# gattia/pyfocusr

Measured on AMD Instinct MI355X. Metric: lowest-k eigenpairs/sec + KNN-correspondence wall-clock, 250k-vertex mesh pair k=5, higher is better.
Workload: dtype f64

## Files before the change

### include/pyfocusr_hip.h

```cpp
#ifndef PYFOCUSR_HIP_H
#define PYFOCUSR_HIP_H

#include <stddef.h>
#include <stdint.h>

#ifdef __cplusplus
extern "C" {
#endif

#define PF_VERSION 1

#define PF_OK 0
#define PF_E_ARG (-1)
#define PF_E_HIP (-2)
#define PF_E_DEGENERATE (-3)
#define PF_E_STATE (-4)
#define PF_E_PERSIST_TIMEOUT (-5)
#define PF_E_INTERNAL (-6)

#define PF_OP_RW 0
#define PF_OP_SYM 1

typedef struct pf_ctx pf_ctx;
typedef struct pf_graph pf_graph;
// ... 97 lines not shown
int pf_orth_end(pf_graph* g, double* h, double* nrm);
int pf_orth_begin2(pf_graph* ga, int32_t w_a, int32_t first_a, int32_t count_a, int32_t normalize_a, pf_graph* gb, int32_t w_b,
                   int32_t first_b, int32_t count_b, int32_t normalize_b);
int pf_orth_cheb2(pf_graph* ga, pf_graph* gb, const int32_t* orth, const int32_t* cheb_i, const double* cheb_d);
int pf_orth_redone(pf_graph* g);
int pf_orth_strict(pf_graph* g, int32_t on);
int pf_orth_device_passes(pf_graph* g, int32_t on);
int pf_orth_split(pf_graph* g, int32_t first2, int32_t split);
int pf_orth_one_launch(int32_t on);
int pf_scale(pf_graph* g, int32_t slot, double alpha);
int pf_combine(pf_graph* g, int32_t src_first, int32_t m, const double* Y, int32_t k, int32_t dst_first);
int pf_resnorm(pf_graph* g, int32_t ax, int32_t x, double lam, double* out);
int pf_gram(pf_graph* g, int32_t first_a, int32_t count_a, int32_t first_b, int32_t count_b, double* out);
int pf_resnorms(pf_graph* g, int32_t ax_first, int32_t x_first, const double* lam, int32_t count, double* out);
int pf_finalize_vectors(pf_graph* g, int32_t first, int32_t count, int32_t from_sym, int32_t minmax,
                        double* out);
int pf_finalize_vectors_begin(pf_graph* g, int32_t first, int32_t count, int32_t from_sym, int32_t minmax, double* out);
int pf_finalize_vectors_end(pf_graph* g);
int pf_final_remap_begin(pf_graph* g, const int32_t* col, const double* sign, int32_t count, double* out);
int pf_host_alloc(size_t bytes, void** out);
int pf_host_free(void* p);
int pf_host_detach(void* p);
int pf_final_rows(pf_graph* g, const int64_t* rows, int64_t n_rows, double* out);
int pf_point_rows(pf_graph* g, const int64_t* rows, int64_t n_rows, double* out);
int pf_spmv_host(pf_graph* g, int32_t op, const double* x, double* y);
int pf_mean_filter(pf_graph* g, const double* values, int32_t ncols, int32_t iterations, double* out);

int pf_knn1(pf_ctx* ctx, const double* ref, int64_t n_ref, const double* qry, int64_t n_qry, int32_t d,
            int64_t* idx_out, double* d2_out);
int pf_knn_mode(pf_ctx* ctx, int32_t mode);
int pf_knn_tree_stats(pf_ctx* ctx, int32_t enable_counting, int64_t* leaves_scanned, int64_t* supers_opened);
int pf_knn_count(pf_ctx* ctx, int32_t enable_counting, int64_t* pairs);
int pf_knn_wave_stats(pf_ctx* ctx, double* sum_us, double* max_us, int64_t* waves, int64_t* max_candidates, double* detail);
int pf_knn(pf_ctx* ctx, const double* ref, int64_t n_ref, const double* qry, int64_t n_qry, int32_t d, int32_t k,
           int64_t* idx_out, double* d2_out);
int pf_knn_topk(pf_ctx* ctx, const double* ref, int64_t n_ref, const double* qry, int64_t n_qry, int32_t d, int32_t k,
                int64_t* idx_out, double* d2_out);
int pf_knn1_graphs(pf_graph* ref_g, pf_graph* qry_g, int32_t d, const int32_t* col_ref, const double* scale_ref,
                   const int32_t* col_qry, const double* scale_qry, int64_t* idx_out, double* d2_out);
int pf_knn1_blocks(pf_ctx* ctx, const double* ref_block, int64_t n_ref, int32_t ref_stride, const double* qry_block,
                   int64_t n_qry, int32_t qry_stride, int32_t d, const int32_t* col_ref, const double* scale_ref,
                   const int32_t* col_qry, const double* scale_qry, int64_t* idx_out, double* d2_out);
int pf_eigsort_costs(pf_graph* g_target, pf_graph* g_source, const int64_t* rows_t, int64_t m_t, const int64_t* rows_s, int64_t m_s,
                     int32_t k, const int32_t* col_t, const double* sign_t, const int32_t* col_s, const double* sign_s, double* out,
                     int64_t* idx_out);
int pf_final_device(pf_graph* g, double** block, int64_t* n_rows, int32_t* n_cols);
int pf_knn_upload(pf_ctx* ctx, const double* ref, int64_t n_ref, const double* qry, int64_t n_qry, int32_t d);
int pf_knn_run(pf_ctx* ctx);
int pf_knn_download(pf_ctx* ctx, int64_t* idx_out, double* d2_out);

int pf_knn1_wide(pf_ctx* ctx, const double* ref, int64_t n_ref, const double* qry, int64_t n_qry, int32_t d,
                 int64_t* idx_out, double* d2_out );
int pf_knn1_wide_count(pf_ctx* ctx, int32_t enable_counting, int64_t* coordinate_pairs);
typedef struct pf_fmap pf_fmap;
int pf_fmap_create(pf_ctx* ctx, const double* phi_t, int64_t n_t, const double* phi_s, int64_t n_s, const double* mass_s,
                   int32_t K, pf_fmap** out);
void pf_fmap_free(pf_fmap* h);
int pf_fmap_set_p2p(pf_fmap* h, const int64_t* T);
int pf_fmap_get_p2p(pf_fmap* h, int64_t* T_out, double* d2_out);
int pf_fmap_project(pf_fmap* h, int32_t k_s, int32_t k_t, double* C_out);
int pf_fmap_convert(pf_fmap* h, const double* C, int32_t k_s, int32_t k_t);
int pf_fmap_zoomout(pf_fmap* h, int32_t k_start, int32_t k_end, int32_t step, int32_t n_iter_at_end, double* C_out);
int pf_fmap_set_samples(pf_fmap* h, const int64_t* S_t, int64_t q_t, const int64_t* S_s, int64_t q_s);
int pf_fmap_zoomout_sampled(pf_fmap* h, int32_t k_start, int32_t k_end, int32_t step, int32_t n_iter_at_end, double* C_out);

int pf_fps(pf_ctx* ctx, const double* points, int64_t n, int32_t d, int64_t m, int64_t start, int64_t* sel_out,
// ... 129 lines not shown
```

### pyfocusr_amd/_hip.py

```python
import atexit
import ctypes as C
import os
import threading
import weakref

import numpy as np

_HERE = os.path.dirname(os.path.abspath(__file__))
LIB_PATH = os.environ.get("PYFOCUSR_HIP_LIB", os.path.join(_HERE, "csrc", "libpyfocusr_hip.so"))

PF_OP_RW = 0
PF_OP_SYM = 1

_f64p = C.POINTER(C.c_double)
_i32p = C.POINTER(C.c_int32)
_i64p = C.POINTER(C.c_int64)


class HipUnavailable(RuntimeError):
    pass


class PfError(RuntimeError):
    def __init__(self, code, msg):
# ... 93 lines not shown
    "pf_eigsort_costs": (C.c_int, [C.c_void_p, C.c_void_p, _i64p, C.c_int64, _i64p, C.c_int64, C.c_int32, _i32p, _f64p, _i32p, _f64p, _f64p,
                                   _i64p]),
    "pf_orth_redone": (C.c_int, [C.c_void_p]),
    "pf_orth_strict": (C.c_int, [C.c_void_p, C.c_int32]),
    "pf_scale": (C.c_int, [C.c_void_p, C.c_int32, C.c_double]),
    "pf_combine": (C.c_int, [C.c_void_p, C.c_int32, C.c_int32, _f64p, C.c_int32, C.c_int32]),
    "pf_resnorm": (C.c_int, [C.c_void_p, C.c_int32, C.c_int32, C.c_double, _f64p]),
    "pf_gram": (C.c_int, [C.c_void_p, C.c_int32, C.c_int32, C.c_int32, C.c_int32, _f64p]),
    "pf_resnorms": (C.c_int, [C.c_void_p, C.c_int32, C.c_int32, _f64p, C.c_int32, _f64p]),
    "pf_finalize_vectors": (C.c_int, [C.c_void_p, C.c_int32, C.c_int32, C.c_int32, C.c_int32, _f64p]),
    "pf_finalize_vectors_begin": (C.c_int, [C.c_void_p, C.c_int32, C.c_int32, C.c_int32, C.c_int32, _f64p]),
    "pf_finalize_vectors_end": (C.c_int, [C.c_void_p]),
    "pf_final_remap_begin": (C.c_int, [C.c_void_p, _i32p, _f64p, C.c_int32, _f64p]),
    "pf_host_alloc": (C.c_int, [C.c_size_t, C.POINTER(C.c_void_p)]),
    "pf_host_free": (C.c_int, [C.c_void_p]),
    "pf_final_rows": (C.c_int, [C.c_void_p, _i64p, C.c_int64, _f64p]),
    "pf_point_rows": (C.c_int, [C.c_void_p, _i64p, C.c_int64, _f64p]),
    "pf_spmv_host": (C.c_int, [C.c_void_p, C.c_int32, _f64p, _f64p]),
    "pf_mean_filter": (C.c_int, [C.c_void_p, _f64p, C.c_int32, C.c_int32, _f64p]),
    "pf_knn1": (C.c_int, [C.c_void_p, _f64p, C.c_int64, _f64p, C.c_int64, C.c_int32, _i64p, _f64p]),
    "pf_knn": (C.c_int, [C.c_void_p, _f64p, C.c_int64, _f64p, C.c_int64, C.c_int32, C.c_int32, _i64p, _f64p]),
    "pf_knn_topk": (C.c_int, [C.c_void_p, _f64p, C.c_int64, _f64p, C.c_int64, C.c_int32, C.c_int32, _i64p, _f64p]),
    "pf_knn1_graphs": (C.c_int, [C.c_void_p, C.c_void_p, C.c_int32, _i32p, _f64p, _i32p, _f64p, _i64p, _f64p]),
    "pf_knn1_blocks": (C.c_int, [C.c_void_p, C.c_void_p, C.c_int64, C.c_int32, C.c_void_p, C.c_int64, C.c_int32, C.c_int32,
                                 _i32p, _f64p, _i32p, _f64p, _i64p, _f64p]),
    "pf_final_device": (C.c_int, [C.c_void_p, C.POINTER(C.c_void_p), _i64p, _i32p]),
    "pf_knn_upload": (C.c_int, [C.c_void_p, _f64p, C.c_int64, _f64p, C.c_int64, C.c_int32]),
    "pf_knn_run": (C.c_int, [C.c_void_p]),
    "pf_knn_download": (C.c_int, [C.c_void_p, _i64p, _f64p]),
    "pf_eigs_smallest": (C.c_int, [C.c_void_p, C.c_int32, C.c_int32, _f64p, _f64p, C.POINTER(C.c_int32), C.POINTER(EigsStats)]),
    "pf_knn_count": (C.c_int, [C.c_void_p, C.c_int32, C.POINTER(C.c_int64)]),
    "pf_knn_wave_stats": (C.c_int, [C.c_void_p, C.POINTER(C.c_double), C.POINTER(C.c_double), C.POINTER(C.c_int64), C.POINTER(C.c_int64),
                                    _f64p]),
    "pf_host_detach": (C.c_int, [C.c_void_p]),
    "pf_orth_device_passes": (C.c_int, [C.c_void_p, C.c_int32]),
    "pf_eigs_smallest_ex": (C.c_int, [C.c_void_p, C.c_int32, C.c_int32, C.c_int32, _f64p, _f64p, _f64p, C.POINTER(C.c_int32),
                                      C.POINTER(EigsStats)]),
    "pf_eigs_smallest2": (C.c_int, [C.c_void_p, C.c_void_p, C.c_int32, C.c_int32, C.c_int32, C.c_int32,
                                    _f64p, _f64p, _f64p, C.POINTER(C.c_int32), C.POINTER(EigsStats),
                                    _f64p, _f64p, _f64p, C.POINTER(C.c_int32), C.POINTER(EigsStats)]),
    "pf_op_step": (C.c_int, [C.c_void_p, C.c_int32, C.c_int32, C.c_int32, C.c_int32, C.c_double, C.c_double, C.c_double]),
    "pf_cheb_steps": (C.c_int, [C.c_void_p, C.c_int32, C.c_int32, C.c_int32, C.c_int32, C.c_int32, C.c_double, C.c_double,
                                C.c_double, C.POINTER(C.c_int32), C.POINTER(C.c_int32)]),
    "pf_axpy": (C.c_int, [C.c_void_p, C.c_int32, C.c_int32, C.c_int32, _f64p]),
    "pf_rows_create": (C.c_int, [C.c_void_p, _i64p, C.c_int64, C.POINTER(C.c_void_p)]),
    "pf_rows_free": (None, [C.c_void_p]),
    "pf_rows_gather": (C.c_int, [C.c_void_p, C.c_int32, _f64p]),
    "pf_rows_scatter": (C.c_int, [C.c_void_p, C.c_int32, _f64p]),
    "pf_rows_gather_dev": (C.c_int, [C.c_void_p, C.c_int32, C.c_void_p]),
    "pf_rows_scatter_dev": (C.c_int, [C.c_void_p, C.c_int32, C.c_void_p]),
    "pf_rows_set_sources": (C.c_int, [C.c_void_p, _i64p]),
    "pf_rows_gather2_dev": (C.c_int, [C.c_void_p, C.c_int32, C.c_int32, C.c_void_p, C.c_int64]),
    "pf_rows_scatter2_dev": (C.c_int, [C.c_void_p, C.c_int32, C.c_int32, C.c_void_p, C.c_int64]),
    "pf_rows_fill": (C.c_int, [C.c_void_p, C.c_int32, C.c_double]),
    "pf_surface_create": (C.c_int, [C.c_void_p, _f64p, C.c_int64, _i32p, C.c_int64, C.c_int32, C.POINTER(C.c_void_p)]),
    "pf_surface_free": (None, [C.c_void_p]),
    "pf_surface_closest": (C.c_int, [C.c_void_p, _f64p, C.c_int64, _f64p, _i32p, _f64p]),
    "pf_surface_distance": (C.c_int, [C.c_void_p, _f64p, C.c_int64, _f64p, _i32p, _f64p]),
    "pf_surface_prepare_signed": (C.c_int, [C.c_void_p, _f64p, _i32p, _i64p]),
    "pf_surface_signed_distance": (C.c_int, [C.c_void_p, _f64p, C.c_int64, _f64p, _i32p, _i32p, _i64p]),
    "pf_surface_prepare_winding": (C.c_int, [C.c_void_p]),
    "pf_surface_winding": (C.c_int, [C.c_void_p, _f64p, C.c_int64, C.c_double, _f64p, _f64p]),
    "pf_surface_raycast": (C.c_int, [C.c_void_p, _f64p, _f64p, C.c_int64, C.c_double, C.c_double, C.c_int32, _f64p, _i32p, _f64p,
                                     _i32p]),
    "pf_surface_vertex_normals": (C.c_int, [C.c_void_p, _f64p]),
    "pf_knn1_wide": (C.c_int, [C.c_void_p, _f64p, C.c_int64, _f64p, C.c_int64, C.c_int32, _i64p, _f64p]),
# ... 320 lines not shown
                child.close()
            self._lib.pf_destroy(self._h)
            self._h = None

    def __del__(self):
        try:
            self.close()
        except Exception:
            pass

    def sync(self):
        _check(self._lib.pf_sync(self._h))

    @property
    def stream_ptr(self):
        return int(self._lib.pf_stream(self._h) or 0)

    def timing_enable(self, on=True):
        _check(self._lib.pf_timing_enable(self._h, int(on)))

    def timing(self, reset=False):
        t = Timing()
        _check(self._lib.pf_timing_get(self._h, C.byref(t), int(bool(reset))))
        return t.as_dict()

    def knn_mode(self, mode):
        _check(self._lib.pf_knn_mode(self._h, int(mode)))

    def knn_count(self, enable_counting=False):
        pairs = C.c_int64()
        _check(self._lib.pf_knn_count(self._h, int(bool(enable_counting)), C.byref(pairs)))
        return int(pairs.value)

    def knn_tree_stats(self, enable_counting=False):
        a, b = C.c_int64(), C.c_int64()
        _check(self._lib.pf_knn_tree_stats(self._h, int(bool(enable_counting)), C.byref(a), C.byref(b)))
        return int(a.value), int(b.value)

    def knn1(self, ref, qry, return_d2=False):
        ref, qry = _same_d(ref, qry)
        idx = np.empty(qry.shape[0], dtype=np.int64)
        d2 = np.empty(qry.shape[0], dtype=np.float64) if return_d2 else None
        _check(self._lib.pf_knn1(self._h, _f64(ref), ref.shape[0], _f64(qry), qry.shape[0], ref.shape[1],
                                 _ptr(idx), _f64(d2)))
        return (idx, d2) if return_d2 else idx

    def knn1_wide(self, ref, qry, return_d2=False):
        ref, qry = _same_d(ref, qry)
        idx = np.empty(qry.shape[0], dtype=np.int64)
        d2 = np.empty(qry.shape[0], dtype=np.float64) if return_d2 else None
        _check(self._lib.pf_knn1_wide(self._h, _f64(ref), ref.shape[0], _f64(qry), qry.shape[0], ref.shape[1],
                                      _ptr(idx), _f64(d2)))
        return (idx, d2) if return_d2 else idx

    def knn1_wide_count(self, enable_counting=False):
        pairs = C.c_int64()
        _check(self._lib.pf_knn1_wide_count(self._h, int(bool(enable_counting)), C.byref(pairs)))
        return int(pairs.value)

    def farthest_point_sampling(self, points, m, start=-1, return_owner=False, return_d2=False):
        pts = _c_f64(points)
        if pts.ndim != 2:
            raise ValueError("points must be an (n, d) array")
        n, m = pts.shape[0], int(m)
        sel = np.empty(max(m, 0), dtype=np.int64)
        owner = np.empty(n, dtype=np.int32) if return_owner else None
# ... 915 lines not shown
```

### pyfocusr_amd/csrc/pf_knn.hip

```cpp
#include <hipcub/hipcub.hpp>

#include <string.h>

#include <algorithm>

#include "pf_internal.h"
#include "pf_wave.h"

namespace {

constexpr int KNN_LDS_DOUBLES = 4096;

struct KnnGrid {
    int a0, a1;
    int r0, r1;
    double lo0, lo1;
    double s0, s1;
};

__device__ __forceinline__ int cell_of(double x, double lo, double scale, int r) {
    const double t = (x - lo) * scale;
    return t > 0.0 ? (t >= (double)r ? r - 1 : (int)t) : 0;
}

__global__ __launch_bounds__(PF_BLOCK) void k_extent(const double* __restrict__ pts, int64_t n, int d, unsigned long long* ext ) {
    __shared__ unsigned long long part[PF_BLOCK / PF_WAVE][32];
    const int wave = threadIdx.x / PF_WAVE;
    for (int a = 0; a < d; ++a) {
        unsigned long long lo = ~0ull, hi = 0ull;
        for (int64_t i = (int64_t)blockIdx.x * PF_BLOCK + threadIdx.x; i < n; i += (int64_t)gridDim.x * PF_BLOCK) {
            const unsigned long long e = enc_f64(pts[i * d + a]);
            lo = e < lo ? e : lo;
            hi = e > hi ? e : hi;
        }
        for (int off = PF_WAVE / 2; off > 0; off >>= 1) {
            const unsigned long long l2 = __shfl_xor(lo, off, PF_WAVE), h2 = __shfl_xor(hi, off, PF_WAVE);
            lo = l2 < lo ? l2 : lo;
            hi = h2 > hi ? h2 : hi;
// ... 19 lines not shown
    }
}

__global__ void k_make_grid(const unsigned long long* __restrict__ ext, int d, int res, KnnGrid* g) {
    if (threadIdx.x | blockIdx.x) return;
    int b0 = 0, b1 = 0;
    double w0 = -1.0, w1 = -1.0;
    for (int a = 0; a < d; ++a) {
        const double e = dec_f64(ext[16 + a]) - dec_f64(ext[a]);
        if (e > w0) {
            w1 = w0;
            b1 = b0;
            w0 = e;
            b0 = a;
        } else if (e > w1) {
            w1 = e;
            b1 = a;
        }
    }
    if (d == 1) {
        b1 = b0;
        w1 = 0.0;
    }
    g->a0 = b0;
    g->a1 = b1;
    g->r0 = res;
    g->r1 = d == 1 ? 1 : res;
    g->lo0 = dec_f64(ext[b0]);
    g->lo1 = dec_f64(ext[b1]);
    g->s0 = (w0 > 0.0 && isfinite(w0)) ? (double)res / w0 : 0.0;
    g->s1 = (d > 1 && w1 > 0.0 && isfinite(w1)) ? (double)res / w1 : 0.0;
}

__device__ __forceinline__ unsigned spread16(unsigned v) {
    v &= 0xffffu;
    v = (v | (v << 8)) & 0x00ff00ffu;
    v = (v | (v << 4)) & 0x0f0f0f0fu;
    v = (v | (v << 2)) & 0x33333333u;
    v = (v | (v << 1)) & 0x55555555u;
    return v;
}

__global__ __launch_bounds__(PF_BLOCK) void k_cell_keys(const double* __restrict__ pts, int64_t n, int d,
                                                        const KnnGrid* __restrict__ gp, int morton, unsigned* __restrict__ keys,
                                                        int32_t* __restrict__ vals, int32_t* __restrict__ hist) {
    const int64_t i = (int64_t)blockIdx.x * PF_BLOCK + threadIdx.x;
    if (i >= n) return;
    const KnnGrid g = *gp;
    const int cx = cell_of(pts[i * d + g.a0], g.lo0, g.s0, g.r0);
    const int cy = cell_of(pts[i * d + g.a1], g.lo1, g.s1, g.r1);
    const unsigned key = morton ? (spread16((unsigned)cx) | (spread16((unsigned)cy) << 1)) : (unsigned)(cy * g.r0 + cx);
    keys[i] = key;
    if (hist) atomicAdd(&hist[key], 1);
    else vals[i] = (int32_t)i;
}

__global__ __launch_bounds__(PF_BLOCK) void k_gather_rows(const double* __restrict__ pts, const int32_t* __restrict__ order,
                                                          int64_t n, int d, double* __restrict__ out) {
    const int64_t i = (int64_t)blockIdx.x * PF_BLOCK + threadIdx.x;
    if (i >= n) return;
    const int64_t src = order[i];
    for (int c = 0; c < d; ++c) out[i * d + c] = pts[src * d + c];
}

__global__ __launch_bounds__(PF_BLOCK) void k_cell_start(const unsigned* __restrict__ keys, int64_t n, int64_t n_cells,
                                                         int32_t* __restrict__ cell_start) {
    const int64_t c = (int64_t)blockIdx.x * PF_BLOCK + threadIdx.x;
    if (c > n_cells) return;
    int64_t lo = 0, hi = n;
    while (lo < hi) {
        const int64_t mid = (lo + hi) >> 1;
        if ((int64_t)keys[mid] < c) lo = mid + 1; else hi = mid;
    }
    cell_start[c] = (int32_t)lo;
}

template <int D>
__device__ __forceinline__ double dist2(const double (&q)[D], const double* __restrict__ r) {
    double s = 0.0;
#pragma unroll
    for (int c = 0; c < D; ++c) {
        const double df = q[c] - r[c];
        const double sq = df * df;
        s = (c == 0) ? sq : s + sq;
// ... 190 lines not shown
                    s = dist2<D>(q, tile + r * D);
                }
                if (s <= bestk[K - 1]) {
                    const int32_t o = tile_idx[r];
                    bool seen = false;
#pragma unroll
                    for (int j = 0; j < K; ++j) seen |= (bidx[j] == o);
                    if (!seen) topk_insert<K>(bestk, bidx, s, o);
                }
            }
        }
        since_refresh += run_e - run_b;
        if (since_refresh >= 4 * KNN_TILE && by1 - by0 >= 8) {
            since_refresh = 0;
            int nx0, nx1, ny0, ny1;
            block_rectangle(nx0, nx1, ny0, ny1);
            bx0 = max(bx0, nx0);
            bx1 = min(bx1, nx1);
            by0 = max(by0, ny0);
            by1 = min(by1, ny1);
        }
    }
    if (mine) {
        const int64_t dst = qry_orig[qi];
#pragma unroll
        for (int j = 0; j < K; ++j) {
            idx_out[dst * K + j] = bidx[j];
            d2_out[dst * K + j] = bestk[j];
        }
    }
}

constexpr int knn_group(int d) { return d <= 4 ? 8 : (d <= 8 ? 4 : 2); }

template <int D, bool COUNT = false>
__global__ __launch_bounds__(PF_BLOCK) void k_knn_coop(const double* __restrict__ soa, int64_t ld, const int32_t* __restrict__ ref_orig,
                                                       const int32_t* __restrict__ cell_start, const double* __restrict__ qry_s,
                                                       const int32_t* __restrict__ qry_orig, int64_t n_qry,
                                                       const KnnGrid* __restrict__ gp, int64_t* __restrict__ idx_out,
                                                       double* __restrict__ d2_out, unsigned long long* __restrict__ visited = nullptr) {
    constexpr int G = knn_group(D);
    unsigned long long seen = 0;
    const unsigned long long t_begin = COUNT ? __builtin_amdgcn_s_memrealtime() : 0ull;
    unsigned long long n_chunks = 0, n_scans = 0, t_scan = 0, t_bounds = 0, n_pass = 0;
    const KnnGrid g = *gp;
    const int lane = threadIdx.x & (PF_WAVE - 1);
    const int64_t group = (int64_t)blockIdx.x * (PF_BLOCK / PF_WAVE) + __builtin_amdgcn_readfirstlane((int)(threadIdx.x / PF_WAVE));
    const int64_t q0 = group * G;
    if (q0 >= n_qry) return;
    const int nq = n_qry - q0 < G ? (int)(n_qry - q0) : G;
    double q[G][D];
    double qx[G], qy[G];
    double best[G];
    int32_t bidx[G];
    int ux0 = 0x7fffffff, ux1 = -1, uy0 = 0x7fffffff, uy1 = -1;
#pragma unroll
    for (int i = 0; i < G; ++i) {
        const int64_t qi = q0 + (i < nq ? i : nq - 1);
#pragma unroll
        for (int c = 0; c < D; ++c) q[i][c] = qry_s[qi * D + c];
        qx[i] = qry_s[qi * D + g.a0];
        qy[i] = qry_s[qi * D + g.a1];
        const int cx = cell_of(qx[i], g.lo0, g.s0, g.r0), cy = cell_of(qy[i], g.lo1, g.s1, g.r1);
        ux0 = min(ux0, cx), ux1 = max(ux1, cx);
        uy0 = min(uy0, cy), uy1 = max(uy1, cy);
        best[i] = INFINITY;
        bidx[i] = 0x7fffffff;
    }
    auto scan_rows = [&](int row_of, int x0, int x1) {
        int32_t b_l = 0, e_l = 0;
        if (row_of >= 0) {
            b_l = cell_start[row_of * g.r0 + x0];
            e_l = cell_start[row_of * g.r0 + x1 + 1];
        }
        int32_t inc = (e_l - b_l + PF_WAVE - 1) >> 6;
#pragma unroll
        for (int off = 1; off < PF_WAVE; off <<= 1) {
            const int32_t up = __shfl_up(inc, off, PF_WAVE);
            if (lane >= off) inc += up;
        }
        const int32_t total = __builtin_amdgcn_readlane(inc, PF_WAVE - 1);
        if constexpr (COUNT) n_chunks += (unsigned long long)total, n_scans += 1ull;
        for (int32_t j = 0; j < total; ++j) {
            const int row = (int)__popcll(__ballot(inc <= j));
            const int32_t first = row > 0 ? __builtin_amdgcn_readlane(inc, row - 1) : 0;
            const int32_t r = __builtin_amdgcn_readlane(b_l, row) + (j - first) * PF_WAVE + lane;
            if constexpr (COUNT) seen += (unsigned long long)__popcll(__ballot(r < __builtin_amdgcn_readlane(e_l, row)));
            if (r < __builtin_amdgcn_readlane(e_l, row)) {
                double x[D];
#pragma unroll
                for (int c = 0; c < D; ++c) x[c] = soa[(int64_t)c * ld + r];
                const int32_t o = ref_orig[r];
                if constexpr (COUNT) {
                    bool pass = false;
#pragma unroll
                    for (int i = 0; i < G; ++i) {
                        double s3 = 0.0;
#pragma unroll
                        for (int c = 0; c < D; ++c)
                            if (c != g.a0 && c != g.a1) s3 += (q[i][c] - x[c]) * (q[i][c] - x[c]);
                        pass = pass || s3 <= best[i];
                    }
                    n_pass += (unsigned long long)__popcll(__ballot(pass));
                }
#pragma unroll
                for (int i = 0; i < G; ++i) {
                    double s = 0.0;
                    constexpr int P = D >= 6 ? D / 2 : D;
#pragma unroll
                    for (int c = 0; c < P; ++c) {
                        const double df = q[i][c] - x[c];
                        const double sq = df * df;
                        s = (c == 0) ? sq : s + sq;
                    }
                    if constexpr (P < D) {
                        if (!__any(s <= best[i])) continue;
#pragma unroll
                        for (int c = P; c < D; ++c) {
                            const double df = q[i][c] - x[c];
                            s = s + df * df;
                        }
                    }
                    if (s < best[i] || (s == best[i] && o < bidx[i])) {
                        best[i] = s;
                        bidx[i] = o;
                    }
                }
            }
        }
    };
    auto bounds = [&](int& bx0, int& bx1, int& by0, int& by1) -> bool {
        bool all = true;
        bx0 = 0x7fffffff, bx1 = -1, by0 = 0x7fffffff, by1 = -1;
#pragma unroll
        for (int i = 0; i < G; ++i) {
            wave_argmin(best[i], bidx[i]);
            all = all && best[i] < INFINITY;
            const double rad = sqrt(best[i]) * (1.0 + 1e-9) + 1e-300;
            double xl = qx[i] - rad, xh = qx[i] + rad, yl = qy[i] - rad, yh = qy[i] + rad;
            xl -= fabs(xl) * 1e-15;
            xh += fabs(xh) * 1e-15;
            yl -= fabs(yl) * 1e-15;
            yh += fabs(yh) * 1e-15;
            bx0 = min(bx0, cell_of(xl, g.lo0, g.s0, g.r0)), bx1 = max(bx1, cell_of(xh, g.lo0, g.s0, g.r0));
            by0 = min(by0, cell_of(yl, g.lo1, g.s1, g.r1)), by1 = max(by1, cell_of(yh, g.lo1, g.s1, g.r1));
        }
        if (!all) bx0 = 0, by0 = 0, bx1 = g.r0 - 1, by1 = g.r1 - 1;
        return all;
    };
    int x0 = 0, x1 = -1, y0 = 0, y1 = -1;
    int rx0 = 0, rx1 = -1, ry0 = 0, ry1 = -1;
    for (int ring = 1; ring <= 4; ++ring) {
        rx0 = max(ux0 - ring, 0), rx1 = min(ux1 + ring, g.r0 - 1);
        ry0 = max(uy0 - ring, 0), ry1 = min(uy1 + ring, g.r1 - 1);
        unsigned long long ta = COUNT ? __builtin_amdgcn_s_memrealtime() : 0ull;
        for (int yb = ry0; yb <= ry1; yb += PF_WAVE) scan_rows(yb + lane <= ry1 ? yb + lane : -1, rx0, rx1);
        unsigned long long tb = COUNT ? __builtin_amdgcn_s_memrealtime() : 0ull;
        const bool all_bounded = bounds(x0, x1, y0, y1);
        if constexpr (COUNT) t_scan += tb - ta, t_bounds += __builtin_amdgcn_s_memrealtime() - tb;
        if (all_bounded) break;
    }
    if (!(x0 >= rx0 && x1 <= rx1 && y0 >= ry0 && y1 <= ry1)) {
        const int mid = min(max((uy0 + uy1) / 2, y0), y1);
        int lo = mid, hi = mid - 1;
        int w = 4;
        while (lo > y0 || hi < y1) {
            const int na = max(min(w, y1 - hi), 0), nb = max(min(w, lo - y0), 0);
            unsigned long long ta = COUNT ? __builtin_amdgcn_s_memrealtime() : 0ull;
            scan_rows(lane < na ? hi + 1 + lane : (lane < na + nb ? lo - 1 - (lane - na) : -1), x0, x1);
            unsigned long long tb = COUNT ? __builtin_amdgcn_s_memrealtime() : 0ull;
            hi += na;
            lo -= nb;
            w = min(2 * w, PF_WAVE / 2);
            int nx0, nx1, ny0, ny1;
            bounds(nx0, nx1, ny0, ny1);
            if constexpr (COUNT) t_scan += tb - ta, t_bounds += __builtin_amdgcn_s_memrealtime() - tb;
            x0 = max(x0, nx0), x1 = min(x1, nx1);
            y0 = max(y0, ny0), y1 = min(y1, ny1);
        }
    }
#pragma unroll
    for (int i = 0; i < G; ++i) {
        if (lane == i && i < nq) {
            const int64_t dst = qry_orig[q0 + i];
            idx_out[dst] = bidx[i];
            d2_out[dst] = best[i];
        }
    }
    if constexpr (COUNT) {
        if (lane == 0 && visited) {
            atomicAdd(visited, seen * (unsigned long long)nq);
            unsigned long long* rec = visited + 8 + 8 * group;
            rec[0] = __builtin_amdgcn_s_memrealtime() - t_begin;
            rec[1] = seen;
            rec[2] = n_chunks;
            rec[3] = n_scans;
            rec[4] = t_scan;
            rec[5] = t_bounds;
            rec[6] = n_pass;
        }
    }
}

constexpr int64_t PF_KNN_SMALL = 16384;
constexpr int knn_small_group(int d) { return d <= 4 ? 8 : 4; }

template <int D>
__global__ __launch_bounds__(PF_BLOCK) void k_knn_small(const double* __restrict__ ref, int64_t n_ref, const double* __restrict__ qry,
                                                        int64_t n_qry, int64_t* __restrict__ idx_out, double* __restrict__ d2_out) {
    constexpr int G = knn_small_group(D);
    const int lane = threadIdx.x & (PF_WAVE - 1);
    const int64_t group = (int64_t)blockIdx.x * (PF_BLOCK / PF_WAVE) + __builtin_amdgcn_readfirstlane((int)(threadIdx.x / PF_WAVE));
    const int64_t q0 = group * G;
    if (q0 >= n_qry) return;
    const int nq = n_qry - q0 < G ? (int)(n_qry - q0) : G;
    double q[G][D], best[G];
    int32_t bidx[G];
#pragma unroll
    for (int i = 0; i < G; ++i) {
        const int64_t qi = q0 + (i < nq ? i : nq - 1);
#pragma unroll
        for (int c = 0; c < D; ++c) q[i][c] = qry[qi * D + c];
        best[i] = INFINITY;
        bidx[i] = 0x7fffffff;
    }
    for (int64_t r = lane; r < n_ref; r += PF_WAVE) {
        double x[D];
#pragma unroll
        for (int c = 0; c < D; ++c) x[c] = ref[r * D + c];
#pragma unroll
        for (int i = 0; i < G; ++i) {
            double s = 0.0;
// ... 11 lines not shown
    }
#pragma unroll
    for (int i = 0; i < G; ++i) {
        wave_argmin(best[i], bidx[i]);
        if (lane == i && i < nq) {
            idx_out[q0 + i] = bidx[i];
            d2_out[q0 + i] = best[i];
        }
    }
}

template <int D>
static int launch_knn_small(pf_ctx* c) {
    const int64_t groups = (c->knn_nqry + knn_small_group(D) - 1) / knn_small_group(D);
    k_knn_small<D><<<(unsigned)((groups + PF_BLOCK / PF_WAVE - 1) / (PF_BLOCK / PF_WAVE)), PF_BLOCK, 0, c->stream>>>(
        c->knn_ref.p, c->knn_nref, c->knn_qry.p, c->knn_nqry, c->knn_idx.p, c->knn_d2.p);
    PF_HIP(hipGetLastError());
    return PF_OK;
}

__global__ __launch_bounds__(PF_BLOCK) void k_gather_rows_soa(const double* __restrict__ pts, const int32_t* __restrict__ order,
                                                              int64_t n, int d, int64_t ld, double* __restrict__ out) {
    const int64_t i = (int64_t)blockIdx.x * PF_BLOCK + threadIdx.x;
    if (i >= n) return;
    const int64_t src = order[i];
    for (int c = 0; c < d; ++c) out[(int64_t)c * ld + i] = pts[src * d + c];
}

template <int D, int K>
int launch_knn_k(pf_ctx* c) {
    constexpr int BS = D <= 6 ? PF_WAVE : PF_BLOCK;
    if constexpr (K == 1 && D <= 9) {
        const int64_t waves = (c->knn_nqry + knn_group(D) - 1) / knn_group(D);
        if (c->knn_count_on) {
            const int64_t words = 8 + 8 * waves;
            PF_HIP(c->knn_visited.grow(c->stream, words));
            c->knn_visited_waves = waves;
            PF_HIP(hipMemsetAsync(c->knn_visited.p, 0, words * sizeof(unsigned long long), c->stream));
            k_knn_coop<D, true><<<(unsigned)((waves + PF_BLOCK / PF_WAVE - 1) / (PF_BLOCK / PF_WAVE)), PF_BLOCK, 0, c->stream>>>(
                c->knn_ref_soa.p, c->knn_ref_ld, c->knn_ref_orig.p, c->knn_cell_start.p, c->knn_qry_s.p, c->knn_qry_orig.p, c->knn_nqry,
                (const KnnGrid*)c->knn_grid, c->knn_idx.p, c->knn_d2.p, c->knn_visited.p);
        } else {
            k_knn_coop<D><<<(unsigned)((waves + PF_BLOCK / PF_WAVE - 1) / (PF_BLOCK / PF_WAVE)), PF_BLOCK, 0, c->stream>>>(
                c->knn_ref_soa.p, c->knn_ref_ld, c->knn_ref_orig.p, c->knn_cell_start.p, c->knn_qry_s.p, c->knn_qry_orig.p, c->knn_nqry,
                (const KnnGrid*)c->knn_grid, c->knn_idx.p, c->knn_d2.p);
        }
    } else {
        k_knn_grid<D, K, BS, 512><<<(unsigned)((c->knn_nqry + BS - 1) / BS), BS, 0, c->stream>>>(
            c->knn_ref_s.p, c->knn_ref_orig.p, c->knn_cell_start.p, c->knn_nref, c->knn_qry_s.p, c->knn_qry_orig.p, c->knn_nqry,
            (const KnnGrid*)c->knn_grid, c->knn_idx.p, c->knn_d2.p);
    }
    PF_HIP(hipGetLastError());
    return PF_OK;
}

template <int D>
int launch_knn(pf_ctx* c) {
    if (c->knn_k == 1) return launch_knn_k<D, 1>(c);
    if constexpr (D <= 4) {
        if (c->knn_k == 2) return launch_knn_k<D, 2>(c);
        if (c->knn_k == 3) return launch_knn_k<D, 3>(c);
        if (c->knn_k == 4) return launch_knn_k<D, 4>(c);
    }
    pf_set_error("pf_knn: k = %d with d = %d is not supported (k <= 4 needs d <= 4)", c->knn_k, D);
    return PF_E_ARG;
}

__global__ __launch_bounds__(PF_BLOCK) void k_bucket_scatter(const unsigned* __restrict__ keys, int64_t n, const int32_t* __restrict__ start,
                                                             int32_t* __restrict__ cursor, unsigned* __restrict__ key_out,
                                                             int32_t* __restrict__ orig_out, const double* __restrict__ pts, int d,
                                                             double* __restrict__ rows_out) {
    const int64_t i = (int64_t)blockIdx.x * PF_BLOCK + threadIdx.x;
    if (i >= n) return;
    const unsigned k = keys[i];
    const int64_t pos = start[k] + atomicAdd(&cursor[k], 1);
    key_out[pos] = k;
    orig_out[pos] = (int32_t)i;
    for (int c = 0; c < d; ++c) rows_out[pos * d + c] = pts[i * d + c];
// ... 163 lines not shown
    unsigned long long h = 0ull;
    if (c->knn_visited.p) {
        PF_HIP(hipMemcpyAsync(&h, c->knn_visited.p, sizeof(h), hipMemcpyDeviceToHost, c->stream));
        PF_HIP(hipStreamSynchronize(c->stream));
    }
    if (pairs) *pairs = (int64_t)h;
    c->knn_count_on = enable_counting != 0;
    return PF_OK;
}

int pf_knn_wave_stats(pf_ctx* c, double* sum_us, double* max_us, int64_t* waves, int64_t* max_candidates, double* detail ) {
    PF_CHECK(c != nullptr, PF_E_ARG, "pf_knn_wave_stats: ctx is NULL");
    const int64_t nw = c->knn_visited.p ? c->knn_visited_waves : 0;
    std::vector<unsigned long long> h((size_t)(8 * nw), 0ull);
    if (nw > 0) {
        PF_HIP(hipMemcpyAsync(h.data(), c->knn_visited.p + 8, sizeof(unsigned long long) * h.size(), hipMemcpyDeviceToHost, c->stream));
        PF_HIP(hipStreamSynchronize(c->stream));
    }
    unsigned long long sum = 0, mx = 0, mc = 0, ch = 0, sc = 0, ts = 0, tb = 0, np = 0;
    for (int64_t w = 0; w < nw; ++w) {
        const unsigned long long* r = h.data() + 8 * w;
        sum += r[0];
        if (r[0] > mx) mx = r[0], mc = r[1];
        ch += r[2], sc += r[3], ts += r[4], tb += r[5], np += r[6];
    }
    if (sum_us) *sum_us = 0.01 * (double)sum;
    if (max_us) *max_us = 0.01 * (double)mx;
    if (waves) *waves = nw;
    if (max_candidates) *max_candidates = (int64_t)mc;
    if (detail) detail[0] = (double)ch, detail[1] = (double)sc, detail[2] = 0.01 * (double)ts, detail[3] = 0.01 * (double)tb, detail[4] = (double)np;
    return PF_OK;
}

int pf_knn_mode(pf_ctx* c, int32_t mode) {
    PF_CHECK(c != nullptr && mode >= 0 && mode <= 2, PF_E_ARG, "pf_knn_mode: bad argument");
    c->knn_mode = mode;
    return PF_OK;
}

int pf_knn_download(pf_ctx* c, int64_t* idx_out, double* d2_out) {
    PF_CHECK(c != nullptr && idx_out != nullptr, PF_E_ARG, "pf_knn_download: NULL argument");
    PF_CHECK(c->knn_done, PF_E_STATE, "pf_knn_download: pf_knn_run has not completed");
    PF_HIP(hipSetDevice(c->device));
    const size_t count = (size_t)c->knn_nqry * c->knn_k;
    const size_t bytes = sizeof(int64_t) * count;
    if (bytes * (d2_out ? 2 : 1) <= ((size_t)8 << 20)) {
        unsigned char* pin = nullptr;
        PF_TRY(pf_pinned_scratch(c, bytes * (d2_out ? 2 : 1), reinterpret_cast<void**>(&pin), 2));
        PF_TRY(pf_copy_by_kernel(c->stream, c->knn_idx.p, pin, bytes));
        if (d2_out) PF_TRY(pf_copy_by_kernel(c->stream, c->knn_d2.p, pin + bytes, bytes));
        PF_HIP(hipStreamSynchronize(c->stream));
        memcpy(idx_out, pin, bytes);
        if (d2_out) memcpy(d2_out, pin + bytes, bytes);
        return PF_OK;
    }
    PF_HIP(hipMemcpyAsync(idx_out, c->knn_idx.p, bytes, hipMemcpyDeviceToHost, c->stream));
    if (d2_out) PF_HIP(hipMemcpyAsync(d2_out, c->knn_d2.p, sizeof(double) * count, hipMemcpyDeviceToHost, c->stream));
    PF_HIP(hipStreamSynchronize(c->stream));
    return PF_OK;
}

int pf_knn(pf_ctx* c, const double* ref, int64_t n_ref, const double* qry, int64_t n_qry, int32_t d, int32_t k,
           int64_t* idx_out, double* d2_out) {
    PF_TRY(knn_upload_k(c, ref, n_ref, qry, n_qry, d, k));
    PF_TRY(pf_knn_run(c));
    return pf_knn_download(c, idx_out, d2_out);
// ... 75 lines not shown
```

Measured before the change: 1016.

## Use Hilbert cell ordering and split spatially spread query groups in cooperative KNN

```diff
diff --git a/include/pyfocusr_hip.h b/include/pyfocusr_hip.h
--- a/include/pyfocusr_hip.h
+++ b/include/pyfocusr_hip.h
@@ -153,6 +153,8 @@
 int pf_knn_tree_stats(pf_ctx* ctx, int32_t enable_counting, int64_t* leaves_scanned, int64_t* supers_opened);
 int pf_knn_count(pf_ctx* ctx, int32_t enable_counting, int64_t* pairs);
 int pf_knn_wave_stats(pf_ctx* ctx, double* sum_us, double* max_us, int64_t* waves, int64_t* max_candidates, double* detail);
+int pf_knn_wave_records(pf_ctx* ctx, uint64_t* records, int64_t max_waves, int64_t* waves);
+int pf_knn_wave_slots(pf_ctx* ctx, int32_t d, int64_t* slots);
 int pf_knn(pf_ctx* ctx, const double* ref, int64_t n_ref, const double* qry, int64_t n_qry, int32_t d, int32_t k,
            int64_t* idx_out, double* d2_out);
 int pf_knn_topk(pf_ctx* ctx, const double* ref, int64_t n_ref, const double* qry, int64_t n_qry, int32_t d, int32_t k,
diff --git a/pyfocusr_amd/_hip.py b/pyfocusr_amd/_hip.py
--- a/pyfocusr_amd/_hip.py
+++ b/pyfocusr_amd/_hip.py
@@ -149,6 +149,8 @@
     "pf_knn_count": (C.c_int, [C.c_void_p, C.c_int32, C.POINTER(C.c_int64)]),
     "pf_knn_wave_stats": (C.c_int, [C.c_void_p, C.POINTER(C.c_double), C.POINTER(C.c_double), C.POINTER(C.c_int64), C.POINTER(C.c_int64),
                                     _f64p]),
+    "pf_knn_wave_records": (C.c_int, [C.c_void_p, C.POINTER(C.c_uint64), C.c_int64, C.POINTER(C.c_int64)]),
+    "pf_knn_wave_slots": (C.c_int, [C.c_void_p, C.c_int32, C.POINTER(C.c_int64)]),
     "pf_host_detach": (C.c_int, [C.c_void_p]),
     "pf_orth_device_passes": (C.c_int, [C.c_void_p, C.c_int32]),
     "pf_eigs_smallest_ex": (C.c_int, [C.c_void_p, C.c_int32, C.c_int32, C.c_int32, _f64p, _f64p, _f64p, C.POINTER(C.c_int32),
@@ -535,6 +537,18 @@
         _check(self._lib.pf_knn_count(self._h, int(bool(enable_counting)), C.byref(pairs)))
         return int(pairs.value)
 
+    def knn_wave_records(self):
+        nw = C.c_int64()
+        _check(self._lib.pf_knn_wave_records(self._h, None, 0, C.byref(nw)))
+        rec = np.zeros((nw.value, 8), dtype=np.uint64)
+        _check(self._lib.pf_knn_wave_records(self._h, _ptr(rec), nw.value, C.byref(nw)))
+        return rec
+
+    def knn_wave_slots(self, d):
+        slots = C.c_int64()
+        _check(self._lib.pf_knn_wave_slots(self._h, int(d), C.byref(slots)))
+        return int(slots.value)
+
     def knn_tree_stats(self, enable_counting=False):
         a, b = C.c_int64(), C.c_int64()
         _check(self._lib.pf_knn_tree_stats(self._h, int(bool(enable_counting)), C.byref(a), C.byref(b)))
diff --git a/pyfocusr_amd/csrc/pf_hilbert.h b/pyfocusr_amd/csrc/pf_hilbert.h
--- /dev/null
+++ b/pyfocusr_amd/csrc/pf_hilbert.h
@@ -0,0 +1,22 @@
+#pragma once
+
+#if defined(__HIPCC__) || defined(__CUDACC__)
+#define PF_HOST_DEVICE __host__ __device__
+#else
+#define PF_HOST_DEVICE
+#endif
+
+PF_HOST_DEVICE inline unsigned pf_hilbert_index(int bits, unsigned x, unsigned y) {
+    unsigned d = 0;
+    for (unsigned s = 1u << (bits - 1); s > 0; s >>= 1) {
+        const unsigned rx = (x & s) ? 1u : 0u, ry = (y & s) ? 1u : 0u;
+        d += s * s * ((3u * rx) ^ ry);
+        if (ry == 0) {
+            if (rx == 1) x ^= s - 1, y ^= s - 1;
+            const unsigned t = x;
+            x = y;
+            y = t;
+        }
+    }
+    return d;
+}
diff --git a/pyfocusr_amd/csrc/pf_knn.hip b/pyfocusr_amd/csrc/pf_knn.hip
--- a/pyfocusr_amd/csrc/pf_knn.hip
+++ b/pyfocusr_amd/csrc/pf_knn.hip
@@ -4,6 +4,7 @@
 
 #include <algorithm>
 
+#include "pf_hilbert.h"
 #include "pf_internal.h"
 #include "pf_wave.h"
 
@@ -89,15 +90,6 @@
     g->s1 = (d > 1 && w1 > 0.0 && isfinite(w1)) ? (double)res / w1 : 0.0;
 }
 
-__device__ __forceinline__ unsigned spread16(unsigned v) {
-    v &= 0xffffu;
-    v = (v | (v << 8)) & 0x00ff00ffu;
-    v = (v | (v << 4)) & 0x0f0f0f0fu;
-    v = (v | (v << 2)) & 0x33333333u;
-    v = (v | (v << 1)) & 0x55555555u;
-    return v;
-}
-
 __global__ __launch_bounds__(PF_BLOCK) void k_cell_keys(const double* __restrict__ pts, int64_t n, int d,
                                                         const KnnGrid* __restrict__ gp, int morton, unsigned* __restrict__ keys,
                                                         int32_t* __restrict__ vals, int32_t* __restrict__ hist) {
@@ -106,7 +98,12 @@
     const KnnGrid g = *gp;
     const int cx = cell_of(pts[i * d + g.a0], g.lo0, g.s0, g.r0);
     const int cy = cell_of(pts[i * d + g.a1], g.lo1, g.s1, g.r1);
-    const unsigned key = morton ? (spread16((unsigned)cx) | (spread16((unsigned)cy) << 1)) : (unsigned)(cy * g.r0 + cx);
+    unsigned key = (unsigned)(cy * g.r0 + cx);
+    if (morton && g.r1 > 1) {
+        int bits = 0;
+        while ((1 << bits) < g.r0) ++bits;
+        key = pf_hilbert_index(bits, (unsigned)cx, (unsigned)cy);
+    }
     keys[i] = key;
     if (hist) atomicAdd(&hist[key], 1);
     else vals[i] = (int32_t)i;
@@ -363,13 +360,15 @@
 }
 
 constexpr int knn_group(int d) { return d <= 4 ? 8 : (d <= 8 ? 4 : 2); }
+constexpr int KNN_SPLIT_SPAN = 16;
 
 template <int D, bool COUNT = false>
 __global__ __launch_bounds__(PF_BLOCK) void k_knn_coop(const double* __restrict__ soa, int64_t ld, const int32_t* __restrict__ ref_orig,
                                                        const int32_t* __restrict__ cell_start, const double* __restrict__ qry_s,
                                                        const int32_t* __restrict__ qry_orig, int64_t n_qry,
                                                        const KnnGrid* __restrict__ gp, int64_t* __restrict__ idx_out,
-                                                       double* __restrict__ d2_out, unsigned long long* __restrict__ visited = nullptr) {
+                                                       double* __restrict__ d2_out, int split_span,
+                                                       unsigned long long* __restrict__ visited = nullptr) {
     constexpr int G = knn_group(D);
     unsigned long long seen = 0;
     const unsigned long long t_begin = COUNT ? __builtin_amdgcn_s_memrealtime() : 0ull;
@@ -384,7 +383,7 @@
     double qx[G], qy[G];
     double best[G];
     int32_t bidx[G];
-    int ux0 = 0x7fffffff, ux1 = -1, uy0 = 0x7fffffff, uy1 = -1;
+    int gx0 = 0x7fffffff, gx1 = -1, gy0 = 0x7fffffff, gy1 = -1;
 #pragma unroll
     for (int i = 0; i < G; ++i) {
         const int64_t qi = q0 + (i < nq ? i : nq - 1);
@@ -393,8 +392,8 @@
         qx[i] = qry_s[qi * D + g.a0];
         qy[i] = qry_s[qi * D + g.a1];
         const int cx = cell_of(qx[i], g.lo0, g.s0, g.r0), cy = cell_of(qy[i], g.lo1, g.s1, g.r1);
-        ux0 = min(ux0, cx), ux1 = max(ux1, cx);
-        uy0 = min(uy0, cy), uy1 = max(uy1, cy);
+        gx0 = min(gx0, cx), gx1 = max(gx1, cx);
+        gy0 = min(gy0, cy), gy1 = max(gy1, cy);
         best[i] = INFINITY;
         bidx[i] = 0x7fffffff;
     }
@@ -460,12 +459,13 @@
             }
         }
     };
-    auto bounds = [&](int& bx0, int& bx1, int& by0, int& by1) -> bool {
+    auto bounds = [&](unsigned act, int& bx0, int& bx1, int& by0, int& by1) -> bool {
         bool all = true;
         bx0 = 0x7fffffff, bx1 = -1, by0 = 0x7fffffff, by1 = -1;
 #pragma unroll
         for (int i = 0; i < G; ++i) {
             wave_argmin(best[i], bidx[i]);
+            if (!((act >> i) & 1u)) continue;
             all = all && best[i] < INFINITY;
             const double rad = sqrt(best[i]) * (1.0 + 1e-9) + 1e-300;
             double xl = qx[i] - rad, xh = qx[i] + rad, yl = qy[i] - rad, yh = qy[i] + rad;
@@ -479,36 +479,49 @@
         if (!all) bx0 = 0, by0 = 0, bx1 = g.r0 - 1, by1 = g.r1 - 1;
         return all;
     };
-    int x0 = 0, x1 = -1, y0 = 0, y1 = -1;
-    int rx0 = 0, rx1 = -1, ry0 = 0, ry1 = -1;
-    for (int ring = 1; ring <= 4; ++ring) {
-        rx0 = max(ux0 - ring, 0), rx1 = min(ux1 + ring, g.r0 - 1);
-        ry0 = max(uy0 - ring, 0), ry1 = min(uy1 + ring, g.r1 - 1);
-        unsigned long long ta = COUNT ? __builtin_amdgcn_s_memrealtime() : 0ull;
-        for (int yb = ry0; yb <= ry1; yb += PF_WAVE) scan_rows(yb + lane <= ry1 ? yb + lane : -1, rx0, rx1);
-        unsigned long long tb = COUNT ? __builtin_amdgcn_s_memrealtime() : 0ull;
-        const bool all_bounded = bounds(x0, x1, y0, y1);
-        if constexpr (COUNT) t_scan += tb - ta, t_bounds += __builtin_amdgcn_s_memrealtime() - tb;
-        if (all_bounded) break;
-    }
-    if (!(x0 >= rx0 && x1 <= rx1 && y0 >= ry0 && y1 <= ry1)) {
-        const int mid = min(max((uy0 + uy1) / 2, y0), y1);
-        int lo = mid, hi = mid - 1;
-        int w = 4;
-        while (lo > y0 || hi < y1) {
-            const int na = max(min(w, y1 - hi), 0), nb = max(min(w, lo - y0), 0);
+    const bool split = nq > 1 && max(gx1 - gx0, gy1 - gy0) + 1 > split_span;
+    const unsigned all_q = (1u << G) - 1u, last = split ? 1u << (nq - 1) : all_q;
+    for (unsigned act = split ? 1u : all_q;; act <<= 1) {
+        int ux0 = 0x7fffffff, ux1 = -1, uy0 = 0x7fffffff, uy1 = -1;
+#pragma unroll
+        for (int i = 0; i < G; ++i) {
+            if (!((act >> i) & 1u)) continue;
+            const int cx = cell_of(qx[i], g.lo0, g.s0, g.r0), cy = cell_of(qy[i], g.lo1, g.s1, g.r1);
+            ux0 = min(ux0, cx), ux1 = max(ux1, cx);
+            uy0 = min(uy0, cy), uy1 = max(uy1, cy);
+        }
+        int x0 = 0, x1 = -1, y0 = 0, y1 = -1;
+        int rx0 = 0, rx1 = -1, ry0 = 0, ry1 = -1;
+        for (int ring = 1; ring <= 4; ++ring) {
+            rx0 = max(ux0 - ring, 0), rx1 = min(ux1 + ring, g.r0 - 1);
+            ry0 = max(uy0 - ring, 0), ry1 = min(uy1 + ring, g.r1 - 1);
             unsigned long long ta = COUNT ? __builtin_amdgcn_s_memrealtime() : 0ull;
-            scan_rows(lane < na ? hi + 1 + lane : (lane < na + nb ? lo - 1 - (lane - na) : -1), x0, x1);
+            for (int yb = ry0; yb <= ry1; yb += PF_WAVE) scan_rows(yb + lane <= ry1 ? yb + lane : -1, rx0, rx1);
             unsigned long long tb = COUNT ? __builtin_amdgcn_s_memrealtime() : 0ull;
-            hi += na;
-            lo -= nb;
-            w = min(2 * w, PF_WAVE / 2);
-            int nx0, nx1, ny0, ny1;
-            bounds(nx0, nx1, ny0, ny1);
+            const bool all_bounded = bounds(act, x0, x1, y0, y1);
             if constexpr (COUNT) t_scan += tb - ta, t_bounds += __builtin_amdgcn_s_memrealtime() - tb;
-            x0 = max(x0, nx0), x1 = min(x1, nx1);
-            y0 = max(y0, ny0), y1 = min(y1, ny1);
-        }
+            if (all_bounded) break;
+        }
+        if (!(x0 >= rx0 && x1 <= rx1 && y0 >= ry0 && y1 <= ry1)) {
+            const int mid = min(max((uy0 + uy1) / 2, y0), y1);
+            int lo = mid, hi = mid - 1;
+            int w = 4;
+            while (lo > y0 || hi < y1) {
+                const int na = max(min(w, y1 - hi), 0), nb = max(min(w, lo - y0), 0);
+                unsigned long long ta = COUNT ? __builtin_amdgcn_s_memrealtime() : 0ull;
+                scan_rows(lane < na ? hi + 1 + lane : (lane < na + nb ? lo - 1 - (lane - na) : -1), x0, x1);
+                unsigned long long tb = COUNT ? __builtin_amdgcn_s_memrealtime() : 0ull;
+                hi += na;
+                lo -= nb;
+                w = min(2 * w, PF_WAVE / 2);
+                int nx0, nx1, ny0, ny1;
+                bounds(act, nx0, nx1, ny0, ny1);
+                if constexpr (COUNT) t_scan += tb - ta, t_bounds += __builtin_amdgcn_s_memrealtime() - tb;
+                x0 = max(x0, nx0), x1 = min(x1, nx1);
+                y0 = max(y0, ny0), y1 = min(y1, ny1);
+            }
+        }
+        if (act >= last) break;
     }
 #pragma unroll
     for (int i = 0; i < G; ++i) {
@@ -529,6 +542,7 @@
             rec[4] = t_scan;
             rec[5] = t_bounds;
             rec[6] = n_pass;
+            rec[7] = ((unsigned long long)(gx1 - gx0 + 1) << 32) | (unsigned long long)(gy1 - gy0 + 1);
         }
     }
 }
@@ -606,6 +620,8 @@
     constexpr int BS = D <= 6 ? PF_WAVE : PF_BLOCK;
     if constexpr (K == 1 && D <= 9) {
         const int64_t waves = (c->knn_nqry + knn_group(D) - 1) / knn_group(D);
+        int split_span = KNN_SPLIT_SPAN;
+        if (const char* ev = getenv("PF_KNN_SPLIT_SPAN")) split_span = atoi(ev);
         if (c->knn_count_on) {
             const int64_t words = 8 + 8 * waves;
             PF_HIP(c->knn_visited.grow(c->stream, words));
@@ -613,11 +629,11 @@
             PF_HIP(hipMemsetAsync(c->knn_visited.p, 0, words * sizeof(unsigned long long), c->stream));
             k_knn_coop<D, true><<<(unsigned)((waves + PF_BLOCK / PF_WAVE - 1) / (PF_BLOCK / PF_WAVE)), PF_BLOCK, 0, c->stream>>>(
                 c->knn_ref_soa.p, c->knn_ref_ld, c->knn_ref_orig.p, c->knn_cell_start.p, c->knn_qry_s.p, c->knn_qry_orig.p, c->knn_nqry,
-                (const KnnGrid*)c->knn_grid, c->knn_idx.p, c->knn_d2.p, c->knn_visited.p);
+                (const KnnGrid*)c->knn_grid, c->knn_idx.p, c->knn_d2.p, split_span, c->knn_visited.p);
         } else {
             k_knn_coop<D><<<(unsigned)((waves + PF_BLOCK / PF_WAVE - 1) / (PF_BLOCK / PF_WAVE)), PF_BLOCK, 0, c->stream>>>(
                 c->knn_ref_soa.p, c->knn_ref_ld, c->knn_ref_orig.p, c->knn_cell_start.p, c->knn_qry_s.p, c->knn_qry_orig.p, c->knn_nqry,
-                (const KnnGrid*)c->knn_grid, c->knn_idx.p, c->knn_d2.p);
+                (const KnnGrid*)c->knn_grid, c->knn_idx.p, c->knn_d2.p, split_span);
         }
     } else {
         k_knn_grid<D, K, BS, 512><<<(unsigned)((c->knn_nqry + BS - 1) / BS), BS, 0, c->stream>>>(
@@ -847,6 +863,33 @@
     return PF_OK;
 }
 
+int pf_knn_wave_records(pf_ctx* c, uint64_t* records, int64_t max_waves, int64_t* waves) {
+    PF_CHECK(c != nullptr && waves != nullptr && (records != nullptr || max_waves == 0) && max_waves >= 0, PF_E_ARG,
+             "pf_knn_wave_records: bad argument");
+    const int64_t nw = c->knn_visited.p ? c->knn_visited_waves : 0;
+    const int64_t take = nw < max_waves ? nw : max_waves;
+    if (take > 0) {
+        PF_HIP(hipMemcpyAsync(records, c->knn_visited.p + 8, sizeof(unsigned long long) * 8 * (size_t)take, hipMemcpyDeviceToHost, c->stream));
+        PF_HIP(hipStreamSynchronize(c->stream));
+    }
+    *waves = nw;
+    return PF_OK;
+}
+
+int pf_knn_wave_slots(pf_ctx* c, int32_t d, int64_t* slots) {
+    PF_CHECK(c != nullptr && slots != nullptr && d >= 1 && d <= 9, PF_E_ARG, "pf_knn_wave_slots: bad argument");
+    PF_HIP(hipSetDevice(c->device));
+    int blocks = 0, cus = 0;
+    const int rc = pf_dispatch_d<1, 9>(d, [&](auto D) -> int {
+        PF_HIP(hipOccupancyMaxActiveBlocksPerMultiprocessor(&blocks, k_knn_coop<D(), false>, PF_BLOCK, 0));
+        return PF_OK;
+    }, "pf_knn_wave_slots: no search for d = %d");
+    PF_TRY(rc);
+    PF_HIP(hipDeviceGetAttribute(&cus, hipDeviceAttributeMultiprocessorCount, c->device));
+    *slots = (int64_t)blocks * cus * (PF_BLOCK / PF_WAVE);
+    return PF_OK;
+}
+
 int pf_knn_mode(pf_ctx* c, int32_t mode) {
     PF_CHECK(c != nullptr && mode >= 0 && mode <= 2, PF_E_ARG, "pf_knn_mode: bad argument");
     c->knn_mode = mode;
```

Result: no change. 1026, median of 4 (+1.0%).
